# barbararoessle/e2e_multi_view_matching

Measured on AMD Instinct MI355X. Metric: image-pairs/sec @1024 kpts + pose AUC@5/10/20deg vs reference, higher is better.
Workload: dtype f16x2 (fp32 operands carried as 2 fp16 planes hi + 2^-11 lo', 22 significant bits, 3 fp16-MFMA products, fp32 accumulate; same 1e-4 / bit-exact-index parity bar); 1 GPU; configs[1]: tuple_size=2 (1 pair per tuple), 1024 keypoints, 256-dim f32 descriptors, GNN 9x1 = 18 layers, 100 Sinkhorn iters, batch 32 tuples/GPU = 32 pairs/GPU, w8pt pose per pair; pairs_per_gpu=32, global_pairs=32, weights=random init (timed), identity-like for the AUC leg, parallelism=tuple-sharded x1

## Files before the change

### e2e_multi_view_matching_amd/csrc/gemm_p2.hip

```cpp
#include <algorithm>
#include <cstdlib>
#include <type_traits>

#include "gemm_p2_core.h"

namespace e2emv {

template <int OUT, bool HAS_R = false>
__global__ __launch_bounds__(512, 1) void gemm_p2_kernel(GemmP2Params p) {
    extern __shared__ __attribute__((aligned(16))) char smem_p2[];

    const int xcd = blockIdx.x & 7, slot = blockIdx.x >> 3, slots = gridDim.x >> 3;
    const int per_xcd = (p.total + 7) / 8;
    const int t_begin = xcd * per_xcd;
    const int t_end = min(t_begin + per_xcd, p.total);
    int tile = t_begin + slot;
    if (tile >= t_end) return;

    const int tid = threadIdx.x, lane = tid & 63;
    const int wave = __builtin_amdgcn_readfirstlane(tid >> 6);
    const int wr = wave >> 1, wc = wave & 1;
    const int l31 = lane & 31, lh = lane >> 5;
    const int nk = p.K / P2_BK, nk1 = p.K1 / P2_BK;

    const __amdgpu_buffer_rsrc_t rsA = __builtin_amdgcn_make_buffer_rsrc(const_cast<uint16_t*>(p.A), 0, (int)p.a_bytes, 0x00020000);
    const __amdgpu_buffer_rsrc_t rsA2 = __builtin_amdgcn_make_buffer_rsrc(const_cast<uint16_t*>(p.A2), 0, (int)p.a2_bytes, 0x00020000);
    const __amdgpu_buffer_rsrc_t rsW = __builtin_amdgcn_make_buffer_rsrc(const_cast<uint16_t*>(p.W), 0, (int)p.w_bytes, 0x00020000);

    const int ld_r = lane >> 3, ld_p = lane & 7;
    unsigned a_vo[4], a2_vo[4], w_vo[4];
    auto setup = [&](int t) {
        const int tm = t / p.tiles_n, tn = t - tm * p.tiles_n;
#pragma unroll
        for (int i = 0; i < 4; ++i) {
            const int row = 32 * wave + 8 * i + ld_r;
            const unsigned c = (unsigned)(ld_p ^ ((row >> 1) & 7));
            const unsigned gm = (unsigned)min(tm * P2_BM + row, p.M - 1);
            a_vo[i] = gm * p.lda_b + c * 16u;
            a2_vo[i] = gm * p.lda2_b + c * 16u;
            const unsigned gn = (unsigned)min(tn * P2_BN + row, p.N - 1);
            w_vo[i] = gn * p.ldw_b + c * 16u;
        }
    };
    auto issue = [&](int buf, int kt, unsigned dep) {
        char* dst = smem_p2 + buf * P2_BUFB + 32 * wave * P2_ROWB;
        if (kt < nk1) {
            const unsigned so = (unsigned)kt * 128u;
#pragma unroll
            for (int i = 0; i < 4; ++i) p2_glds16(rsA, dst + i * 1024, a_vo[i] + dep, so);
        } else {
            const unsigned so = (unsigned)(kt - nk1) * 128u;
#pragma unroll
            for (int i = 0; i < 4; ++i) p2_glds16(rsA2, dst + i * 1024, a2_vo[i] + dep, so);
        }
        const unsigned sw = (unsigned)kt * 128u;
#pragma unroll
        for (int i = 0; i < 4; ++i) p2_glds16(rsW, dst + P2_TILEB + i * 1024, w_vo[i] + dep, sw);
    };

    const int swz = (l31 >> 1) & 7;
    p2_f32x16 acc[4][2];



    int ld_tile = tile, ld_kt = 0;
    bool ld_valid = true;
    auto advance = [&]() {
        if (ld_kt + 1 < nk) { ++ld_kt; return; }
        if (ld_tile + slots < t_end) {
            ld_tile += slots;
            ld_kt = 0;
            setup(ld_tile);
        } else {
            ld_valid = false;
        }
    };
    setup(tile);
    issue(0, 0, 0u);
    advance();
    const bool issue_first = wave >= 4;
    const bool overlap = nk >= 3;
    const bool has_e = p.EA != nullptr || (HAS_R && p.ER != nullptr);
    int e_run = 0, cur_kt = 0;
    int ev = 0, ev_next = 0;
    auto fetch_e = [&](int t) {
        int v = 0;
        if (has_e) {
            const int tm_ = t / p.tiles_n, tn_ = t - tm_ * p.tiles_n;
            const int erow = tm_ * 4 + wr;
            const int nb1 = nk1 >> 1, nb = (nk + 1) >> 1;
            if (erow * 64 < p.M) {
                if (lane < nb) {
                    if (p.EA) v = lane < nb1 ? p.EA[erow * p.eld_a + lane] : (p.EA2 ? p.EA2[erow * p.eld_a2 + lane - nb1] : 0);
                } else if (HAS_R && p.ER && lane >= 32 && lane < 36) {
                    const int cb = tn_ * 4 + wc * 2 + (lane & 1);
                    if (cb < p.eld_r) {
                        if (lane < 34) v = p.ER[erow * p.eld_r + cb];
                        else if (p.AR) v = __builtin_bit_cast(int, p.AR[erow * p.eld_r + cb]);
                    }
                }
            }
        }
        return v;
    };
    ev = fetch_e(tile);
    int since = 8;
    bool ahead = false;
    int buf = 0;
    auto step = [&](auto FIRST) {
        if (since == 0 && ahead) asm volatile("s_waitcnt vmcnt(40)" ::: "memory");
        else if (since <= 1 && overlap) asm volatile("s_waitcnt vmcnt(32)" ::: "memory");
        else asm volatile("s_waitcnt vmcnt(0)" ::: "memory");
        asm volatile("s_waitcnt lgkmcnt(0)\n\ts_barrier" ::: "memory");
        if (has_e) {
            const int e_step = p.EA ? __builtin_amdgcn_readlane(ev, cur_kt >> 1) : 0;
            if (!decltype(FIRST)::value && e_step != e_run) {
                asm volatile("s_nop 15");
                const int d = e_run - e_step;
                const float f = d < -126 ? 0.f : p2_exp2i(d);
#pragma unroll
                for (int j = 0; j < 4; ++j)
#pragma unroll
                    for (int i = 0; i < 2; ++i)
#pragma unroll
                        for (int r = 0; r < 16; ++r) acc[j][i][r] *= f;
            }
            e_run = e_step;
            if (nk >= 4 && tile + slots < t_end) {
                if (cur_kt == 2) ev_next = fetch_e(tile + slots);
                if (cur_kt == 3) asm volatile("" : "+v"(ev_next));
            }
        }
        ++cur_kt;
        const bool ldv = ld_valid && !(since == 0 && ahead);
        if (issue_first && ldv) issue(buf ^ 1, ld_kt, 0u);
        gp_kstep<decltype(FIRST)::value>(smem_p2, buf, wr, wc, l31, lh, acc);
        if (!issue_first && ldv) {
            unsigned dep = 0;
            asm("" : "+v"(dep) : "v"(acc[3][1]));
            issue(buf ^ 1, ld_kt, dep);
        }
        if (ldv) advance();
        if (since == 0) ahead = false;
        ++since;
        buf ^= 1;
    };
    for (;;) {
        step(std::true_type{});
        for (int kt = 1; kt < nk; ++kt) step(std::false_type{});
        if (overlap && ld_valid) {
            asm volatile("s_waitcnt lgkmcnt(0)\n\ts_barrier" ::: "memory");
            unsigned dep = 0;
            asm("" : "+v"(dep) : "v"(acc[3][1]));
            issue(buf ^ 1, ld_kt, dep);
            advance();
            ahead = true;
        }
        cur_kt = 0;
        if (has_e && nk < 4 && tile + slots < t_end) ev_next = fetch_e(tile + slots);
        gp_acc_fence(acc);
        gp_epilogue<OUT, HAS_R>(p, smem_p2, acc, wave, tile / p.tiles_n, tile % p.tiles_n, e_run, ev);
        ev = ev_next;
        since = overlap ? 0 : 8;
        tile += slots;
        if (tile >= t_end) break;
    }
}

int fill_gemm_p2_params(e2emv_ctx* ctx, const GemmP2Args& a, GemmP2Params& p) {
    if (a.M <= 0 || a.N <= 0 || a.K <= 0) return set_err(ctx, E2EMV_ESHAPE, "gemm_p2: empty problem");
    const int K1 = a.A2 ? a.K1 : a.K;
    if (a.K % 32 || K1 % 32 || K1 <= 0 || K1 > a.K || (K1 < a.K && !a.A2))
        return set_err(ctx, E2EMV_ESHAPE, "gemm_p2: K=%d K1=%d must be multiples of 32", a.K, K1);
    if (!a.A || !a.W || a.lda % 32 || a.lda < K1 || (a.A2 && (a.lda2 % 32 || a.lda2 < a.K - K1)))
        return set_err(ctx, E2EMV_ESHAPE, "gemm_p2: operand planes need whole 32-column blocks (lda=%lld lda2=%lld)", (long long)a.lda, (long long)a.lda2);
    if ((uintptr_t)a.A % 16 || (a.A2 && (uintptr_t)a.A2 % 16) || (uintptr_t)a.W % 16 || (a.bias && (uintptr_t)a.bias % 16) || (a.Rp && (uintptr_t)a.Rp % 16))
        return set_err(ctx, E2EMV_ESHAPE, "gemm_p2: operands must be 16-byte aligned");
    if (a.Rp && (a.ldr % 32 || a.ldr < a.N)) return set_err(ctx, E2EMV_ESHAPE, "gemm_p2: residual planes need ldr %% 32 == 0");
    const int64_t a_bytes = (int64_t)a.M * a.lda * 4, a2_bytes = a.A2 ? (int64_t)a.M * a.lda2 * 4 : 16, w_bytes = (int64_t)a.N * a.K * 4;
    if (a_bytes >= ((int64_t)1 << 31) || a2_bytes >= ((int64_t)1 << 31) || w_bytes >= ((int64_t)1 << 31))
        return set_err(ctx, E2EMV_ESHAPE, "gemm_p2: operand larger than 2 GB (M=%d lda=%lld): 32-bit byte offsets", a.M, (long long)a.lda);
    p = GemmP2Params{};
    p.A = a.A; p.A2 = a.A2 ? a.A2 : a.A; p.W = a.W;
    p.a_bytes = (unsigned)a_bytes; p.a2_bytes = (unsigned)(a.A2 ? a2_bytes : a_bytes); p.w_bytes = (unsigned)w_bytes;
    p.lda_b = (unsigned)(a.lda * 4); p.lda2_b = (unsigned)((a.A2 ? a.lda2 : a.lda) * 4); p.ldw_b = (unsigned)(a.K * 4);
    p.bias = a.bias; p.Rp = a.Rp; p.ldr = a.ldr;
// ... 61 lines not shown
```

### e2e_multi_view_matching_amd/csrc/gemm_p2_core.h

```cpp
#pragma once
#include <type_traits>

#include "p2.h"

namespace e2emv {

typedef __attribute__((ext_vector_type(16))) float p2_f32x16;

constexpr int P2_BM = 256, P2_BN = 256, P2_BK = 32;
constexpr int P2_ROWB = 128;
constexpr int P2_TILEB = P2_BM * P2_ROWB;
constexpr int P2_BUFB = 2 * P2_TILEB;
constexpr int P2_SLABB = 32 * 32 * 4;
constexpr int P2_LDSB = 2 * P2_BUFB + 8 * P2_SLABB;

struct GemmP2Params {
    const uint16_t* A;
    const uint16_t* A2;
    const uint16_t* W;
    unsigned a_bytes, a2_bytes, w_bytes;
    unsigned lda_b, lda2_b, ldw_b;
    const float* bias;
    const uint16_t* Rp;
    float* C32;
    uint16_t* Cp;
    uint16_t* Vt;
    int64_t ldc, ldr;
    int M, N, K, K1;
    int tiles_n, total, relu;
    float out_scale;
    float col_scale[3];
    int n_rows, heads;
    const int* EA;
    const int* EA2;
    const int* ER;
    int* EC;
    int* EVt;
    const float* AR;
    float* AC;
    int eld_a, eld_a2, eld_r, eld_c;
    float bias_amax;
    unsigned* stats;
    char* dummy;
};

__device__ __forceinline__ int gp_lane_now() {
    int l;
    asm volatile("v_mbcnt_lo_u32_b32 %0, -1, 0\n\tv_mbcnt_hi_u32_b32 %0, -1, %0" : "=v"(l));
    return l;
}

int fill_gemm_p2_params(e2emv_ctx* ctx, const GemmP2Args& a, GemmP2Params& p);

__device__ __forceinline__ void gp_mfma(p2_f32x16& c, p2_f16x8 a, p2_f16x8 b) {
    asm volatile("v_mfma_f32_32x32x16_f16 %0, %1, %2, %0" : "+v"(c) : "v"(a), "v"(b));
}
__device__ __forceinline__ void gp_mfma0(p2_f32x16& c, p2_f16x8 a, p2_f16x8 b) {
    asm volatile("v_mfma_f32_32x32x16_f16 %0, %1, %2, 0" : "=&v"(c) : "v"(a), "v"(b));
}
__device__ __forceinline__ unsigned gp_pk_mul(unsigned x, unsigned k) {
    unsigned d;
    asm volatile("v_pk_mul_f16 %0, %1, %2" : "=v"(d) : "v"(x), "v"(k));
    return d;
}

__device__ __forceinline__ float gp_amax3(float a, float x, float y) {
    asm("v_max3_f32 %0, %0, |%1|, |%2|" : "+v"(a) : "v"(x), "v"(y));
    return a;
}
__device__ __forceinline__ void gp_relu2x8(p2_f32x4& v0, p2_f32x4& v1, int on) {
    float a = v0[0], b = v0[1], c = v0[2], d = v0[3], e = v1[0], f = v1[1], g = v1[2], h = v1[3];
    asm("s_cmp_eq_u32 %8, 0\n\t"
        "s_cbranch_scc1 1f\n\t"
        "v_add_f32_e64 %0, %0, |%0|\n\t"
        "v_add_f32_e64 %1, %1, |%1|\n\t"
        "v_add_f32_e64 %2, %2, |%2|\n\t"
        "v_add_f32_e64 %3, %3, |%3|\n\t"
        "v_add_f32_e64 %4, %4, |%4|\n\t"
        "v_add_f32_e64 %5, %5, |%5|\n\t"
        "v_add_f32_e64 %6, %6, |%6|\n\t"
        "v_add_f32_e64 %7, %7, |%7|\n"
        "1:"
        : "+v"(a), "+v"(b), "+v"(c), "+v"(d), "+v"(e), "+v"(f), "+v"(g), "+v"(h) : "s"(on) : "scc");
    v0 = p2_f32x4{a, b, c, d};
    v1 = p2_f32x4{e, f, g, h};
}
__device__ __forceinline__ p2_f32x2 gp_join_scaled(unsigned hi, unsigned lo) {
    float x0, x1;
    asm("v_fma_mix_f32 %0, %2, %4, %3 op_sel_hi:[1,0,1]\n\tv_fma_mix_f32 %1, %2, %4, %3 op_sel:[1,0,1] op_sel_hi:[1,0,1]"
        : "=&v"(x0), "=&v"(x1) : "v"(lo), "v"(hi), "s"(1.f / 2048.f));
    return {x0, x1};
}
template <bool SCALED>
__device__ __forceinline__ void gp_split8(const p2_f32x4& a0, const p2_f32x4& a1, const p2_f32x4& b0, const p2_f32x4& b1, p2_u32x4& hi, p2_u32x4& lo) {
    const p2_f32x2 q0 = {a0[0], a0[1]}, q1 = {a0[2], a0[3]}, q2 = {a1[0], a1[1]}, q3 = {a1[2], a1[3]};
    const unsigned h0 = __builtin_bit_cast(unsigned, __builtin_convertvector(q0, p2_f16x2)), h1 = __builtin_bit_cast(unsigned, __builtin_convertvector(q1, p2_f16x2));
    const unsigned h2 = __builtin_bit_cast(unsigned, __builtin_convertvector(q2, p2_f16x2)), h3 = __builtin_bit_cast(unsigned, __builtin_convertvector(q3, p2_f16x2));
    unsigned l0, l1, l2, l3;
    asm("v_fma_mixlo_f16 %0, %4, %16, %8 op_sel_hi:[1,0,0]\n\t"
        "v_fma_mixlo_f16 %1, %5, %16, %10 op_sel_hi:[1,0,0]\n\t"
        "v_fma_mixlo_f16 %2, %6, %16, %12 op_sel_hi:[1,0,0]\n\t"
        "v_fma_mixlo_f16 %3, %7, %16, %14 op_sel_hi:[1,0,0]\n\t"
        "v_fma_mixhi_f16 %0, %4, %16, %9 op_sel:[1,0,0] op_sel_hi:[1,0,0]\n\t"
        "v_fma_mixhi_f16 %1, %5, %16, %11 op_sel:[1,0,0] op_sel_hi:[1,0,0]\n\t"
        "v_fma_mixhi_f16 %2, %6, %16, %13 op_sel:[1,0,0] op_sel_hi:[1,0,0]\n\t"
        "v_fma_mixhi_f16 %3, %7, %16, %15 op_sel:[1,0,0] op_sel_hi:[1,0,0]\n\t"
        "s_nop 1"
        : "=&v"(l0), "=&v"(l1), "=&v"(l2), "=&v"(l3)
        : "v"(h0), "v"(h1), "v"(h2), "v"(h3), "v"(b0[0]), "v"(b0[1]), "v"(b0[2]), "v"(b0[3]), "v"(b1[0]), "v"(b1[1]), "v"(b1[2]), "v"(b1[3]),
          "s"(SCALED ? -2048.f : -1.f));
    hi = p2_u32x4{h0, h1, h2, h3};
    lo = p2_u32x4{l0, l1, l2, l3};
}

template <bool first_step>
__device__ __forceinline__ void gp_kstep(const char* smem, int buf, int wr, int wc, int l31, int lh, p2_f32x16 (&acc)[4][2]) {
    const int swz = (l31 >> 1) & 7;
    const char* xs = smem + buf * P2_BUFB + (wr * 64 + l31) * P2_ROWB;
    const char* ws = smem + buf * P2_BUFB + P2_TILEB + (wc * 128 + l31) * P2_ROWB;
    auto rd_x = [&](int ks, int t, int pl) { return *reinterpret_cast<const p2_f16x8*>(xs + t * 32 * P2_ROWB + (((4 * pl + 2 * ks + lh) ^ swz) << 4)); };
    auto rd_w = [&](int ks, int j, int pl) { return *reinterpret_cast<const p2_f16x8*>(ws + j * 32 * P2_ROWB + (((4 * pl + 2 * ks + lh) ^ swz) << 4)); };
    p2_f16x8 xb[2][2][2];
    p2_f16x8 wb[2][2];
    unsigned k2048 = 0x10001000u;
    asm volatile("" : "+v"(k2048));
#pragma unroll
    for (int t = 0; t < 2; ++t)
#pragma unroll
        for (int pl = 0; pl < 2; ++pl) xb[0][t][pl] = rd_x(0, t, pl);
    wb[0][1] = rd_w(0, 0, 1);
    wb[0][0] = rd_w(0, 0, 0);
    __builtin_amdgcn_sched_barrier(0);
#pragma unroll
    for (int g = 0; g < 8; ++g) {
        const int ks = g >> 2, j = g & 3, gp = g & 1;
        const p2_u32x4 wh = __builtin_bit_cast(p2_u32x4, wb[gp][0]);
        p2_u32x4 w2u;
        const bool z = first_step && ks == 0;
        if (z) gp_mfma0(acc[j][0], wb[gp][1], xb[ks][0][0]); else gp_mfma(acc[j][0], wb[gp][1], xb[ks][0][0]);
#pragma unroll
        for (int e = 0; e < 4; ++e) w2u[e] = gp_pk_mul(wh[e], k2048);
        __builtin_amdgcn_sched_barrier(0);
        if (z) gp_mfma0(acc[j][1], wb[gp][1], xb[ks][1][0]); else gp_mfma(acc[j][1], wb[gp][1], xb[ks][1][0]);
        if (g < 7) {
            wb[gp ^ 1][1] = rd_w((g + 1) >> 2, (g + 1) & 3, 1);
            wb[gp ^ 1][0] = rd_w((g + 1) >> 2, (g + 1) & 3, 0);
        }
        __builtin_amdgcn_sched_barrier(0);
        const p2_f16x8 w2 = __builtin_bit_cast(p2_f16x8, w2u);
        gp_mfma(acc[j][0], w2, xb[ks][0][1]);
        if (ks == 0 && j == 2) { xb[1][0][0] = rd_x(1, 0, 0); xb[1][1][0] = rd_x(1, 1, 0); }
        __builtin_amdgcn_sched_barrier(0);
        gp_mfma(acc[j][1], w2, xb[ks][1][1]);
        if (ks == 0 && j == 3) { xb[1][0][1] = rd_x(1, 0, 1); xb[1][1][1] = rd_x(1, 1, 1); }
        __builtin_amdgcn_sched_barrier(0);
        gp_mfma(acc[j][0], wb[gp][0], xb[ks][0][0]);
        __builtin_amdgcn_sched_barrier(0);
        gp_mfma(acc[j][1], wb[gp][0], xb[ks][1][0]);
        __builtin_amdgcn_sched_barrier(0);
    }
}

__device__ __forceinline__ void gp_acc_fence(p2_f32x16 (&acc)[4][2]) {
    asm volatile("s_nop 15" : "+v"(acc[0][0]), "+v"(acc[0][1]), "+v"(acc[1][0]), "+v"(acc[1][1]), "+v"(acc[2][0]), "+v"(acc[2][1]), "+v"(acc[3][0]), "+v"(acc[3][1]));
}

template <int OUT, bool HAS_R, bool RLDS = false>
__device__ __forceinline__ void gp_epilogue(const GemmP2Params& p, char* smem, const p2_f32x16 (&acc)[4][2], int wave, int tm, int tn, int e_run, int ev) {
    static_assert(!RLDS || (HAS_R && OUT == P2_OUT_PLANES), "the LDS residual ring belongs to the plane epilogue with a residual");
    const int lane = gp_lane_now();
    const int wr = wave >> 1, wc = wave & 1;
    const int l31 = lane & 31, lh = lane >> 5;
    char* sl = smem + 2 * P2_BUFB + wave * P2_SLABB;
    const int o_r = lane >> 2, o_c = (lane & 3) * 8;
    const int o_z = o_r & 7;
    const float cs = OUT == P2_OUT_QKV ? p.col_scale[min(tn, 2)] : 1.f;
    char* dummy = p.dummy + lane * 64;
    const float os = p.out_scale * p2_exp2i(e_run);
    const int erow = tm * 4 + wr;
    float rsc[2] = {1.f, 1.f};
    float osc[2] = {1.f, 1.f};
    float iosc[2] = {1.f, 1.f};
    float amx[2][2] = {{0.f, 0.f}, {0.f, 0.f}};
    if ((OUT != P2_OUT_F32 && (p.EC || p.EVt)) || (HAS_R && p.ER)) {
#pragma unroll
        for (int ch = 0; ch < 2; ++ch) {
            const int cb = tn * 4 + wc * 2 + ch;
            int er = 0;
            float ar = 0.f;
            if (HAS_R && p.ER) {
                er = __builtin_amdgcn_readlane(ev, 32 + ch);
                ar = p.AR ? __builtin_bit_cast(float, __builtin_amdgcn_readlane(ev, 34 + ch)) : 65536.f * p2_exp2i(er);
            }
            rsc[ch] = p2_exp2i(er);
            int* E = (OUT == P2_OUT_QKV && tn == 2) ? p.EVt : p.EC;
            if (OUT == P2_OUT_F32 || !E) continue;
            float am = 0.f, am1 = 0.f;
#pragma unroll
            for (int i = 0; i < 2; ++i)
#pragma unroll
                for (int jj = 0; jj < 2; ++jj)
#pragma unroll
                    for (int r = 0; r < 16; r += 4) {
                        am = gp_amax3(am, acc[2 * ch + jj][i][r], acc[2 * ch + jj][i][r + 1]);
                        am1 = gp_amax3(am1, acc[2 * ch + jj][i][r + 2], acc[2 * ch + jj][i][r + 3]);
                    }
            am = p2_wave_max(fmaxf(am, am1));
            const float bound = am * os + p.bias_amax + ar;
            const int e = p2_pick_exponent(bound * cs);
            osc[ch] = p2_exp2i(-e);
            iosc[ch] = p2_exp2i(e);
            const int ecb = (OUT == P2_OUT_QKV && tn == 2) ? wc * 2 + ch : cb;
            const int eld = (OUT == P2_OUT_QKV && tn == 2) ? 4 : p.eld_c;
            if (lane == 0 && erow * 64 < p.M && ecb < eld) {
                E[erow * eld + ecb] = e;
                if (e != 0 && p.stats) atomicAdd(p.stats, 1u);
            }
        }
    }
    const unsigned sw0 = (unsigned)(uintptr_t)(__attribute__((address_space(3))) char*)sl + (unsigned)(l31 * 128 + ((lh ^ (l31 & 7)) << 4));
    auto slab_write = [&](int i, int j) {
        unsigned a = sw0;
        asm volatile("" : "+v"(a));
#pragma unroll
        for (int g = 0; g < 4; ++g) {
            p2_f32x4 v;
#pragma unroll
            for (int e = 0; e < 4; ++e) v[e] = acc[j][i][4 * g + e];
            typedef __attribute__((address_space(3))) p2_f32x4* lds_f32x4_t;
            *reinterpret_cast<lds_f32x4_t>((uintptr_t)(a ^ (32u * g))) = v;
        }
    };
    if (OUT == P2_OUT_QKV && tn == 2) {
        const int dl0 = lane >> 2, q = lane & 3;
        const int rb = 16 * (q >> 1) + 4 * (q & 1);
        float vb[4][2];
#pragma unroll
        for (int j = 0; j < 4; ++j)
#pragma unroll
            for (int pass = 0; pass < 2; ++pass) {
                const int n = tn * P2_BN + wc * 128 + j * 32 + dl0 + 16 * pass;
                vb[j][pass] = (p.bias && n < p.N) ? p.bias[n] : 0.f;
            }
        const unsigned vt_rd0 = (unsigned)(uintptr_t)(__attribute__((address_space(3))) char*)sl
                                + (unsigned)(rb * 128 + ((((dl0 >> 2) ^ (rb & 7)) << 4) | ((dl0 & 3) << 2)));
        const int64_t row2 = 2 * (int64_t)p.n_rows;
        uint16_t* const vt_lane = p.Vt + dl0 * row2 + q * 8;
#pragma unroll
        for (int i = 0; i < 2; ++i) {
            const int m0 = tm * P2_BM + wr * 64 + i * 32;
            const int img = m0 / p.n_rows, key0 = m0 - img * p.n_rows;
            const int64_t off_i = (int64_t)img * p.heads * 64 * row2 + (key0 >> 5) * 64;
#pragma unroll
            for (int j = 0; j < 4; ++j) {
                slab_write(i, j);
                const float f = cs * osc[j >> 1], of = os * f;
#pragma unroll
                for (int pass = 0; pass < 2; ++pass) {
                    const int dl = dl0 + 16 * pass;
                    unsigned a0 = vt_rd0 ^ (pass ? 64u : 0u);
                    asm volatile("" : "+v"(a0));
                    float v[8];
#pragma unroll
                    for (int t = 0; t < 4; ++t) {
// ... 41 lines not shown
    }
    auto rl_issue = [&](int bb) {
        if constexpr (RLDS) {
            const int i = bb >> 2, j = bb & 3;
            const unsigned m0 = (unsigned)(tm * P2_BM + wr * 64 + i * 32);
            const unsigned so = m0 * (unsigned)p.ldr * 4u + (unsigned)(tn * 8 + wc * 4 + j) * 128u;
            asm volatile("" ::: "memory");
#pragma unroll
            for (int q = 0; q < 4; ++q) p2_glds16(rsR, rl_base + (bb & 3) * 4096 + q * 1024, rl_vo, so + (unsigned)q * 8u * (unsigned)p.ldr * 4u);
            asm volatile("" ::: "memory");
        }
    };
    if constexpr (RLDS) {
#pragma unroll
        for (int bb = 0; bb < 4; ++bb) rl_issue(bb);
    }
    p2_f32x4 rv[2][2][2];
    p2_u32x4 rr[RREG ? 2 : 1][2][2];
    const int row0 = tm * P2_BM + wr * 64 + o_r, col0 = tn * P2_BN + wc * 128 + o_c;
    const int rows_left = p.M - row0;
    const int64_t rstep = (OUT == P2_OUT_F32 ? 16 : 32) * p.ldc;
    float* const c32_t = OUT == P2_OUT_F32 ? p.C32 + (int64_t)row0 * p.ldc + col0 : nullptr;
    uint16_t* const cp_t = OUT == P2_OUT_F32 ? nullptr : p.Cp + p2_index(row0, col0, p.ldc);
    const bool relu = OUT != P2_OUT_QKV && p.relu;
    const bool fold = relu && OUT == P2_OUT_PLANES && !HAS_R;
    const float unfold = relu && !fold ? 0.5f : 1.f;
    auto stage = [&](auto BB) {
        constexpr int b = decltype(BB)::value;
        constexpr int i = b >> 2, j = b & 3;
        slab_write(i, j);
        if (RREG) load_bias(b & 1, j);
        const uint16_t* rcol = nullptr;
        if constexpr (RREG) {
            const int nc = min(col0 + j * 32, p.N - 8);
            rcol = p.Rp + ((nc >> 5) * 64 + (nc & 31));
        }
#pragma unroll
        for (int pass = 0; pass < 2; ++pass) {
            const int r = o_r + 16 * pass;
            const int c0 = 2 * (lane & 3);
            rv[b & 1][pass][0] = *reinterpret_cast<const p2_f32x4*>(sl + r * 128 + ((c0 ^ o_z) << 4));
            rv[b & 1][pass][1] = *reinterpret_cast<const p2_f32x4*>(sl + r * 128 + (((c0 + 1) ^ o_z) << 4));
            if constexpr (RREG) {
                int m = min(row0 + i * 32 + 16 * pass, p.M - 1);
                const uint16_t* rp = rcol + (int64_t)m * (2 * p.ldr);
                rr[b & 1][pass][0] = *reinterpret_cast<const p2_u32x4*>(rp);
                rr[b & 1][pass][1] = *reinterpret_cast<const p2_u32x4*>(rp + 32);
            }
        }
    };
    auto finish = [&](auto BB) {
        constexpr int b = decltype(BB)::value;
        constexpr int i = b >> 2, j = b & 3;
        const bool col_ok = col0 + j * 32 < p.N;
        const float fa = OUT == P2_OUT_F32 ? 1.f : cs * osc[j >> 1] * (fold ? 0.5f : 1.f);
        float osf = os, rsf = 1.f;
        if constexpr (HAS_R) rsf = rsc[j >> 1];
        p2_u32x4 rq[2][2];
        if constexpr (RLDS) {
            constexpr int CNT[8] = {12, 16, 20, 24, 28, 24, 20, 16};
            asm volatile("s_waitcnt vmcnt(%0)" :: "n"(CNT[b]) : "memory");
            const unsigned sw = (((unsigned)o_r >> 1) & 1u) << 2;
#pragma unroll
            for (int pass = 0; pass < 2; ++pass) {
                const char* rp_ = rl_base + (b & 3) * 4096 + (o_r + 16 * pass) * 128;
                rq[pass][0] = *reinterpret_cast<const p2_u32x4*>(rp_ + ((((unsigned)lane & 3u) ^ sw) << 4));
                rq[pass][1] = *reinterpret_cast<const p2_u32x4*>(rp_ + (((4u + ((unsigned)lane & 3u)) ^ sw) << 4));
// ... 77 lines not shown
```

### e2e_multi_view_matching_amd/csrc/gemm_p2c.hip

```cpp
#include <algorithm>
#include <cstdlib>

#include "gemm_p2_core.h"

namespace e2emv {

constexpr int P2C_MAX_STAGES = 4, P2C_MAX_TILES = 16;
constexpr int P2C_INDEP = P2_CHAIN_INDEP;

struct GemmP2ChainParams {
    GemmP2Params st[P2C_MAX_STAGES];
    int kind[P2C_MAX_STAGES];
    int dep_kt[P2C_MAX_STAGES];
    int first[P2C_MAX_STAGES + 1];
    int n_stages, row_blocks;
    int t_info[P2C_MAX_TILES];
};

__global__ __launch_bounds__(512, 1) void gemm_p2_chain_kernel(GemmP2ChainParams cp_by_value) {
    extern __shared__ __attribute__((aligned(16))) char smem_p2c[];
    (void)cp_by_value;
    const GemmP2ChainParams& cp = *(const GemmP2ChainParams*)(const __attribute__((address_space(4))) GemmP2ChainParams*)__builtin_amdgcn_kernarg_segment_ptr();

    const int wave = __builtin_amdgcn_readfirstlane(threadIdx.x >> 6);
    const int wr = wave >> 1, wc = wave & 1;
    int l31 = 0, lh = 0;
    unsigned rc_t = 0;
    const int nst = cp.n_stages, tpr = cp.first[nst];
    const int n_my = (cp.row_blocks - (int)blockIdx.x + (int)gridDim.x - 1) / (int)gridDim.x;
    const int total = n_my * tpr;
    if (total <= 0) return;
    auto is_hard = [&](int f) { return f > 0 && (cp.t_info[f % tpr] & (1 << 16)) != 0; };

    unsigned a_base = 0, w_base = 0;
    unsigned lda_l = 0, ldw_l = 0;
    __amdgpu_buffer_rsrc_t rsA, rsA2, rsW;
    int nk_l = 0, nk1_l = 0;
    auto setup = [&](int f) {
        const int rbi = f / tpr, r = f - rbi * tpr, ti = cp.t_info[r], s = ti & 255;
        const int tm = (int)blockIdx.x + rbi * (int)gridDim.x, tn = (ti >> 8) & 255;
        const GemmP2Params& q = cp.st[s];
        rsA = __builtin_amdgcn_make_buffer_rsrc(const_cast<uint16_t*>(q.A), 0, (int)q.a_bytes, 0x00020000);
        rsA2 = __builtin_amdgcn_make_buffer_rsrc(const_cast<uint16_t*>(q.A2), 0, (int)q.a2_bytes, 0x00020000);
        rsW = __builtin_amdgcn_make_buffer_rsrc(const_cast<uint16_t*>(q.W), 0, (int)q.w_bytes, 0x00020000);
        nk_l = q.K / P2_BK;
        nk1_l = q.K1 / P2_BK;
        lda_l = q.lda_b;
        ldw_l = q.ldw_b;
        a_base = ((unsigned)tm * P2_BM + 32u * wave) * lda_l;
        w_base = ((unsigned)tn * P2_BN + 32u * wave) * ldw_l;
    };
    auto lane_rc = [&]() {
        const unsigned ln = (unsigned)gp_lane_now(), ld_r = ln >> 3, ld_p = ln & 7;
        return ld_r | ((ld_p ^ (ld_r >> 1)) * 16u) << 8;
    };
    auto issue = [&](int buf, int kt, unsigned rc) {
        char* dst = smem_p2c + buf * P2_BUFB + 32 * wave * P2_ROWB;
        const unsigned ld_r = rc & 255u, c16 = rc >> 8;
        const unsigned a0 = __umul24(ld_r, lda_l) + c16, a1 = a0 ^ 64u, w0 = __umul24(ld_r, ldw_l) + c16, w1 = w0 ^ 64u;
// ... 18 lines not shown
        p2_glds16(rsW, dst + P2_TILEB + 3072, w1, sw + 3 * w_step);
    };

    typedef int p2c_i4 __attribute__((ext_vector_type(4)));
    typedef int p2c_i2 __attribute__((ext_vector_type(2)));
    auto sload4 = [](const int* p) {
        p2c_i4 r;
        asm volatile("s_load_dwordx4 %0, %1, 0x0\n\ts_waitcnt lgkmcnt(0)" : "=&s"(r) : "s"(p) : "memory");
        return r;
    };
    auto sload2 = [](const int* p) {
        p2c_i2 r;
        asm volatile("s_load_dwordx2 %0, %1, 0x0\n\ts_waitcnt lgkmcnt(0)" : "=&s"(r) : "s"(p) : "memory");
        return r;
    };
    auto pack4 = [](p2c_i4 v) { return (unsigned)((v[0] & 255) | (v[1] & 255) << 8 | (v[2] & 255) << 16 | (v[3] & 255) << 24); };
    auto fetch_ew = [&](int f, bool low, bool high, unsigned long long old) {
        const int rbi = f / tpr, r = f - rbi * tpr, ti = cp.t_info[r], s = ti & 255;
        const int erow = ((int)blockIdx.x + rbi * (int)gridDim.x) * 4 + wr;
        const GemmP2Params& q = cp.st[s];
        if (!q.EA) return 0ull;
        const int nb1 = (q.K1 / P2_BK) >> 1, nb = (q.K / P2_BK + 1) >> 1;
        unsigned lo = (unsigned)old, hi = (unsigned)(old >> 32);
        if (low) lo = pack4(sload4(q.EA + erow * q.eld_a));
        if (high) {
            hi = 0;
            if (nb1 == 8) hi = pack4(sload4(q.EA + erow * q.eld_a + 4));
            else if (nb > nb1 && q.EA2) hi = pack4(sload4(q.EA2 + erow * q.eld_a2));
        }
        return (unsigned long long)hi << 32 | lo;
    };
    auto e_of = [](unsigned long long ew, int kb) { return (int)(signed char)(ew >> (8 * kb)); };

    p2_f32x16 acc[4][2];
    int lf = 0, lkt = 0;
    bool ld_valid = true, ld_blocked = false;
    auto advance = [&]() {
        if (__builtin_expect(lkt + 1 < nk_l, 1)) { ++lkt; return; }
        if (lf + 1 >= total) { ld_valid = false; return; }
        if (is_hard(lf + 1)) { ld_blocked = true; return; }
        ++lf;
        lkt = 0;
        setup(lf);
    };
    setup(0);
    issue(0, 0, lane_rc());
    advance();
    unsigned long long ew = fetch_ew(0, true, true, 0), ew_next = 0;
    int er_c[2] = {0, 0}, ar_c[2] = {0, 0};
    const bool issue_first = wave >= 4;
    int e_run = 0, cur_kt = 0;
    int since = 8;
    bool ahead = false;
    int buf = 0;
    bool has_e = false, soft = false, prefetch_next = false;
    int f = 0;
    auto step = [&](auto FIRST) {
        if (since == 0 && ahead) asm volatile("s_waitcnt vmcnt(40)" ::: "memory");
        else if (since <= 1) asm volatile("s_waitcnt vmcnt(32)" ::: "memory");
        else asm volatile("s_waitcnt vmcnt(0)" ::: "memory");
        asm volatile("s_waitcnt lgkmcnt(0)\n\ts_barrier" ::: "memory");
        if (has_e && (cur_kt & 1) == 0) {
            if (__builtin_expect(soft && cur_kt == 4, 0)) {
                asm volatile("s_dcache_inv\n\tbuffer_inv sc0\n\ts_waitcnt lgkmcnt(0)" ::: "memory");
                ew = fetch_ew(f, false, true, ew);
            }
            const int e_step = e_of(ew, cur_kt >> 1);
            if (!decltype(FIRST)::value && __builtin_expect(e_step != e_run, 0)) {
                asm volatile("s_nop 15");
                const int d = e_run - e_step;
                const float fs = d < -126 ? 0.f : p2_exp2i(d);
#pragma unroll
                for (int j = 0; j < 4; ++j)
#pragma unroll
                    for (int i = 0; i < 2; ++i)
#pragma unroll
                        for (int r = 0; r < 16; ++r) acc[j][i][r] *= fs;
            }
            e_run = e_step;
            if (__builtin_expect(cur_kt == 2, 0)) {
                if (prefetch_next) ew_next = fetch_ew(f + 1, true, true, 0);
                const int rr_ = f % tpr, ti_ = cp.t_info[rr_], s_ = ti_ & 255;
                const GemmP2Params& q_ = cp.st[s_];
                if ((cp.kind[s_] & 4) && q_.ER) {
                    const int erow = ((int)blockIdx.x + (f / tpr) * (int)gridDim.x) * 4 + wr;
                    const int cb = ((ti_ >> 8) & 255) * 4 + wc * 2;
                    const p2c_i2 e2 = sload2(q_.ER + erow * q_.eld_r + cb);
                    er_c[0] = e2[0]; er_c[1] = e2[1];
                    if (q_.AR) {
                        const p2c_i2 a2 = sload2(reinterpret_cast<const int*>(q_.AR) + erow * q_.eld_r + cb);
                        ar_c[0] = a2[0]; ar_c[1] = a2[1];
                    }
                }
            }
        }
        ++cur_kt;
        const bool ldv = ld_valid && !ld_blocked && !(since == 0 && ahead);
        if (issue_first && ldv) issue(buf ^ 1, lkt, rc_t);
        gp_kstep<decltype(FIRST)::value>(smem_p2c, buf, wr, wc, l31, lh, acc);
        if (!issue_first && ldv) {
            unsigned rc = rc_t;
            asm("" : "+v"(rc) : "v"(acc[3][1]));
            issue(buf ^ 1, lkt, rc);
        }
        if (ldv) advance();
        if (since == 0) ahead = false;
        ++since;
        buf ^= 1;
    };
    for (f = 0; f < total; ++f) {
        const int rbi = f / tpr, r = f - rbi * tpr, ti = cp.t_info[r], s = ti & 255;
        const int tm = (int)blockIdx.x + rbi * (int)gridDim.x, tn = (ti >> 8) & 255;
        const GemmP2Params& q = cp.st[s];
        const int nk = q.K / P2_BK;
        {
            const int ln = gp_lane_now();
            l31 = ln & 31;
            lh = ln >> 5;
            rc_t = lane_rc();
        }
        has_e = q.EA != nullptr || ((cp.kind[s] & 4) && q.ER != nullptr);
        soft = f > 0 && (ti & (1 << 17)) != 0;
        prefetch_next = f + 1 < total && !is_hard(f + 1);
        step(std::true_type{});
        for (int kt = 1; kt < nk; ++kt) step(std::false_type{});
        if (ld_valid && !ld_blocked) {
            asm volatile("s_waitcnt lgkmcnt(0)\n\ts_barrier" ::: "memory");
            unsigned rc = lane_rc();
            asm("" : "+v"(rc) : "v"(acc[3][1]));
            issue(buf ^ 1, lkt, rc);
            advance();
            ahead = true;
        }
        cur_kt = 0;
        gp_acc_fence(acc);
        int ev = 0;
        if ((cp.kind[s] & 4) && q.ER) {
            asm("v_writelane_b32 %0, %1, 32\n\tv_writelane_b32 %0, %2, 33\n\tv_writelane_b32 %0, %3, 34\n\tv_writelane_b32 %0, %4, 35"
                : "+v"(ev) : "s"(er_c[0]), "s"(er_c[1]), "s"(ar_c[0]), "s"(ar_c[1]));
        }
        switch (cp.kind[s]) {
            case P2_OUT_PLANES: gp_epilogue<P2_OUT_PLANES, false>(q, smem_p2c, acc, wave, tm, tn, e_run, ev); break;
            case P2_OUT_PLANES | 4:
                if (ld_blocked) {
                    asm volatile("s_waitcnt lgkmcnt(0)\n\ts_barrier" ::: "memory");
                    gp_epilogue<P2_OUT_PLANES, true, true>(q, smem_p2c, acc, wave, tm, tn, e_run, ev);
                } else {
                    gp_epilogue<P2_OUT_PLANES, true>(q, smem_p2c, acc, wave, tm, tn, e_run, ev);
                }
                break;
            case P2_OUT_QKV: gp_epilogue<P2_OUT_QKV, false>(q, smem_p2c, acc, wave, tm, tn, e_run, ev); break;
            default: gp_epilogue<P2_OUT_F32, false>(q, smem_p2c, acc, wave, tm, tn, e_run, ev); break;
        }
        ew = ew_next;
        since = 0;
        if (ld_blocked) {
            asm volatile("s_waitcnt vmcnt(0) lgkmcnt(0)\n\ts_barrier\n\tbuffer_inv sc0" ::: "memory");
            ld_blocked = false;
            ++lf;
            lkt = 0;
            setup(lf);
            asm volatile("s_dcache_inv\n\ts_waitcnt lgkmcnt(0)" ::: "memory");
// ... 53 lines not shown
```

Measured before the change: 3321 pairs/s.

## Switch P2 GEMM core from 32x32x16 to 16x16x32 MFMA tiles

Replaces the 32x32x16 f16 MFMA with 16x16x32, changing the accumulator layout to an 8x4 array of f32x4 fragments. The k-step LDS read pattern, swizzle and scheduling are rewritten to match, and the epilogue amax and slab writes are adapted to the new fragment layout. The aim is better MFMA throughput and latency hiding by covering the full 32-deep K slice in one instruction per fragment, at the cost of more MFMA issues, more LDS fragment reads and a different register allocation. It also adds a readfirstlane on the picked exponent and a profiling script that reports effective clock per kernel.

```diff
diff --git a/e2e_multi_view_matching_amd/csrc/gemm_p2.hip b/e2e_multi_view_matching_amd/csrc/gemm_p2.hip
--- a/e2e_multi_view_matching_amd/csrc/gemm_p2.hip
+++ b/e2e_multi_view_matching_amd/csrc/gemm_p2.hip
@@ -20,7 +20,6 @@
     const int tid = threadIdx.x, lane = tid & 63;
     const int wave = __builtin_amdgcn_readfirstlane(tid >> 6);
     const int wr = wave >> 1, wc = wave & 1;
-    const int l31 = lane & 31, lh = lane >> 5;
     const int nk = p.K / P2_BK, nk1 = p.K1 / P2_BK;
 
     const __amdgpu_buffer_rsrc_t rsA = __builtin_amdgcn_make_buffer_rsrc(const_cast<uint16_t*>(p.A), 0, (int)p.a_bytes, 0x00020000);
@@ -58,8 +57,7 @@
         for (int i = 0; i < 4; ++i) p2_glds16(rsW, dst + P2_TILEB + i * 1024, w_vo[i] + dep, sw);
     };
 
-    const int swz = (l31 >> 1) & 7;
-    p2_f32x16 acc[4][2];
+    p2_acc_t acc;
 
 
 
@@ -119,11 +117,11 @@
                 const int d = e_run - e_step;
                 const float f = d < -126 ? 0.f : p2_exp2i(d);
 #pragma unroll
-                for (int j = 0; j < 4; ++j)
-#pragma unroll
-                    for (int i = 0; i < 2; ++i)
-#pragma unroll
-                        for (int r = 0; r < 16; ++r) acc[j][i][r] *= f;
+                for (int j = 0; j < P2_ACC_J; ++j)
+#pragma unroll
+                    for (int i = 0; i < P2_ACC_I; ++i)
+#pragma unroll
+                        for (int r = 0; r < 4; ++r) acc[j][i][r] *= f;
             }
             e_run = e_step;
             if (nk >= 4 && tile + slots < t_end) {
@@ -134,10 +132,10 @@
         ++cur_kt;
         const bool ldv = ld_valid && !(since == 0 && ahead);
         if (issue_first && ldv) issue(buf ^ 1, ld_kt, 0u);
-        gp_kstep<decltype(FIRST)::value>(smem_p2, buf, wr, wc, l31, lh, acc);
+        gp_kstep<decltype(FIRST)::value>(smem_p2, buf, wr, wc, lane, acc);
         if (!issue_first && ldv) {
             unsigned dep = 0;
-            asm("" : "+v"(dep) : "v"(acc[3][1]));
+            asm("" : "+v"(dep) : "v"(acc[P2_ACC_J - 1][P2_ACC_I - 1]));
             issue(buf ^ 1, ld_kt, dep);
         }
         if (ldv) advance();
@@ -151,7 +149,7 @@
         if (overlap && ld_valid) {
             asm volatile("s_waitcnt lgkmcnt(0)\n\ts_barrier" ::: "memory");
             unsigned dep = 0;
-            asm("" : "+v"(dep) : "v"(acc[3][1]));
+            asm("" : "+v"(dep) : "v"(acc[P2_ACC_J - 1][P2_ACC_I - 1]));
             issue(buf ^ 1, ld_kt, dep);
             advance();
             ahead = true;
diff --git a/e2e_multi_view_matching_amd/csrc/gemm_p2_core.h b/e2e_multi_view_matching_amd/csrc/gemm_p2_core.h
--- a/e2e_multi_view_matching_amd/csrc/gemm_p2_core.h
+++ b/e2e_multi_view_matching_amd/csrc/gemm_p2_core.h
@@ -5,7 +5,8 @@
 
 namespace e2emv {
 
-typedef __attribute__((ext_vector_type(16))) float p2_f32x16;
+constexpr int P2_ACC_J = 8, P2_ACC_I = 4;
+typedef p2_f32x4 p2_acc_t[P2_ACC_J][P2_ACC_I];
 
 constexpr int P2_BM = 256, P2_BN = 256, P2_BK = 32;
 constexpr int P2_ROWB = 128;
@@ -52,11 +53,11 @@
 
 int fill_gemm_p2_params(e2emv_ctx* ctx, const GemmP2Args& a, GemmP2Params& p);
 
-__device__ __forceinline__ void gp_mfma(p2_f32x16& c, p2_f16x8 a, p2_f16x8 b) {
-    asm volatile("v_mfma_f32_32x32x16_f16 %0, %1, %2, %0" : "+v"(c) : "v"(a), "v"(b));
-}
-__device__ __forceinline__ void gp_mfma0(p2_f32x16& c, p2_f16x8 a, p2_f16x8 b) {
-    asm volatile("v_mfma_f32_32x32x16_f16 %0, %1, %2, 0" : "=&v"(c) : "v"(a), "v"(b));
+__device__ __forceinline__ void gp_mfma(p2_f32x4& c, p2_f16x8 a, p2_f16x8 b) {
+    asm volatile("v_mfma_f32_16x16x32_f16 %0, %1, %2, %0" : "+v"(c) : "v"(a), "v"(b));
+}
+__device__ __forceinline__ void gp_mfma0(p2_f32x4& c, p2_f16x8 a, p2_f16x8 b) {
+    asm volatile("v_mfma_f32_16x16x32_f16 %0, %1, %2, 0" : "=&v"(c) : "v"(a), "v"(b));
 }
 __device__ __forceinline__ unsigned gp_pk_mul(unsigned x, unsigned k) {
     unsigned d;
@@ -114,63 +115,71 @@
 }
 
 template <bool first_step>
-__device__ __forceinline__ void gp_kstep(const char* smem, int buf, int wr, int wc, int l31, int lh, p2_f32x16 (&acc)[4][2]) {
-    const int swz = (l31 >> 1) & 7;
-    const char* xs = smem + buf * P2_BUFB + (wr * 64 + l31) * P2_ROWB;
-    const char* ws = smem + buf * P2_BUFB + P2_TILEB + (wc * 128 + l31) * P2_ROWB;
-    auto rd_x = [&](int ks, int t, int pl) { return *reinterpret_cast<const p2_f16x8*>(xs + t * 32 * P2_ROWB + (((4 * pl + 2 * ks + lh) ^ swz) << 4)); };
-    auto rd_w = [&](int ks, int j, int pl) { return *reinterpret_cast<const p2_f16x8*>(ws + j * 32 * P2_ROWB + (((4 * pl + 2 * ks + lh) ^ swz) << 4)); };
-    p2_f16x8 xb[2][2][2];
+__device__ __forceinline__ void gp_kstep(const char* smem, int buf, int wr, int wc, int lane, p2_acc_t& acc) {
+    const int l15 = lane & 15, lq = lane >> 4;
+    const int swz = l15 >> 1;
+    const char* xs = smem + buf * P2_BUFB + (wr * 64 + l15) * P2_ROWB;
+    const char* ws = smem + buf * P2_BUFB + P2_TILEB + (wc * 128 + l15) * P2_ROWB;
+    auto rd_x = [&](int t, int pl) { return *reinterpret_cast<const p2_f16x8*>(xs + t * 16 * P2_ROWB + (((4 * pl + lq) ^ swz) << 4)); };
+    auto rd_w = [&](int j, int pl) { return *reinterpret_cast<const p2_f16x8*>(ws + j * 16 * P2_ROWB + (((4 * pl + lq) ^ swz) << 4)); };
+    p2_f16x8 xb[4][2];
     p2_f16x8 wb[2][2];
     unsigned k2048 = 0x10001000u;
     asm volatile("" : "+v"(k2048));
-#pragma unroll
-    for (int t = 0; t < 2; ++t)
-#pragma unroll
-        for (int pl = 0; pl < 2; ++pl) xb[0][t][pl] = rd_x(0, t, pl);
-    wb[0][1] = rd_w(0, 0, 1);
-    wb[0][0] = rd_w(0, 0, 0);
+    xb[0][0] = rd_x(0, 0);
+    wb[0][1] = rd_w(0, 1);
+    xb[1][0] = rd_x(1, 0);
+    wb[0][0] = rd_w(0, 0);
+    xb[2][0] = rd_x(2, 0);
+    xb[3][0] = rd_x(3, 0);
     __builtin_amdgcn_sched_barrier(0);
 #pragma unroll
     for (int g = 0; g < 8; ++g) {
-        const int ks = g >> 2, j = g & 3, gp = g & 1;
+        const int gp = g & 1;
         const p2_u32x4 wh = __builtin_bit_cast(p2_u32x4, wb[gp][0]);
         p2_u32x4 w2u;
-        const bool z = first_step && ks == 0;
-        if (z) gp_mfma0(acc[j][0], wb[gp][1], xb[ks][0][0]); else gp_mfma(acc[j][0], wb[gp][1], xb[ks][0][0]);
+        if (first_step) gp_mfma0(acc[g][0], wb[gp][1], xb[0][0]); else gp_mfma(acc[g][0], wb[gp][1], xb[0][0]);
 #pragma unroll
         for (int e = 0; e < 4; ++e) w2u[e] = gp_pk_mul(wh[e], k2048);
+        if (g == 0) { xb[0][1] = rd_x(0, 1); xb[1][1] = rd_x(1, 1); }
         __builtin_amdgcn_sched_barrier(0);
-        if (z) gp_mfma0(acc[j][1], wb[gp][1], xb[ks][1][0]); else gp_mfma(acc[j][1], wb[gp][1], xb[ks][1][0]);
+        if (first_step) gp_mfma0(acc[g][1], wb[gp][1], xb[1][0]); else gp_mfma(acc[g][1], wb[gp][1], xb[1][0]);
         if (g < 7) {
-            wb[gp ^ 1][1] = rd_w((g + 1) >> 2, (g + 1) & 3, 1);
-            wb[gp ^ 1][0] = rd_w((g + 1) >> 2, (g + 1) & 3, 0);
-        }
+            wb[gp ^ 1][1] = rd_w(g + 1, 1);
+            wb[gp ^ 1][0] = rd_w(g + 1, 0);
+        }
+        __builtin_amdgcn_sched_barrier(0);
+        if (first_step) gp_mfma0(acc[g][2], wb[gp][1], xb[2][0]); else gp_mfma(acc[g][2], wb[gp][1], xb[2][0]);
+        if (g == 0) { xb[2][1] = rd_x(2, 1); xb[3][1] = rd_x(3, 1); }
+        __builtin_amdgcn_sched_barrier(0);
+        if (first_step) gp_mfma0(acc[g][3], wb[gp][1], xb[3][0]); else gp_mfma(acc[g][3], wb[gp][1], xb[3][0]);
         __builtin_amdgcn_sched_barrier(0);
         const p2_f16x8 w2 = __builtin_bit_cast(p2_f16x8, w2u);
-        gp_mfma(acc[j][0], w2, xb[ks][0][1]);
-        if (ks == 0 && j == 2) { xb[1][0][0] = rd_x(1, 0, 0); xb[1][1][0] = rd_x(1, 1, 0); }
-        __builtin_amdgcn_sched_barrier(0);
-        gp_mfma(acc[j][1], w2, xb[ks][1][1]);
-        if (ks == 0 && j == 3) { xb[1][0][1] = rd_x(1, 0, 1); xb[1][1][1] = rd_x(1, 1, 1); }
-        __builtin_amdgcn_sched_barrier(0);
-        gp_mfma(acc[j][0], wb[gp][0], xb[ks][0][0]);
-        __builtin_amdgcn_sched_barrier(0);
-        gp_mfma(acc[j][1], wb[gp][0], xb[ks][1][0]);
-        __builtin_amdgcn_sched_barrier(0);
-    }
-}
-
-__device__ __forceinline__ void gp_acc_fence(p2_f32x16 (&acc)[4][2]) {
-    asm volatile("s_nop 15" : "+v"(acc[0][0]), "+v"(acc[0][1]), "+v"(acc[1][0]), "+v"(acc[1][1]), "+v"(acc[2][0]), "+v"(acc[2][1]), "+v"(acc[3][0]), "+v"(acc[3][1]));
+#pragma unroll
+        for (int i = 0; i < 4; ++i) {
+            gp_mfma(acc[g][i], w2, xb[i][1]);
+            __builtin_amdgcn_sched_barrier(0);
+        }
+#pragma unroll
+        for (int i = 0; i < 4; ++i) {
+            gp_mfma(acc[g][i], wb[gp][0], xb[i][0]);
+            __builtin_amdgcn_sched_barrier(0);
+        }
+    }
+}
+
+__device__ __forceinline__ void gp_acc_fence(p2_acc_t& acc) {
+    asm volatile("s_nop 15" : "+v"(acc[0][0]), "+v"(acc[0][1]), "+v"(acc[0][2]), "+v"(acc[0][3]), "+v"(acc[1][0]), "+v"(acc[1][1]), "+v"(acc[1][2]), "+v"(acc[1][3]),
+                              "+v"(acc[2][0]), "+v"(acc[2][1]), "+v"(acc[2][2]), "+v"(acc[2][3]), "+v"(acc[3][0]), "+v"(acc[3][1]), "+v"(acc[3][2]), "+v"(acc[3][3]));
+    asm volatile("s_nop 15" : "+v"(acc[4][0]), "+v"(acc[4][1]), "+v"(acc[4][2]), "+v"(acc[4][3]), "+v"(acc[5][0]), "+v"(acc[5][1]), "+v"(acc[5][2]), "+v"(acc[5][3]),
+                              "+v"(acc[6][0]), "+v"(acc[6][1]), "+v"(acc[6][2]), "+v"(acc[6][3]), "+v"(acc[7][0]), "+v"(acc[7][1]), "+v"(acc[7][2]), "+v"(acc[7][3]));
 }
 
 template <int OUT, bool HAS_R, bool RLDS = false>
-__device__ __forceinline__ void gp_epilogue(const GemmP2Params& p, char* smem, const p2_f32x16 (&acc)[4][2], int wave, int tm, int tn, int e_run, int ev) {
+__device__ __forceinline__ void gp_epilogue(const GemmP2Params& p, char* smem, const p2_acc_t& acc, int wave, int tm, int tn, int e_run, int ev) {
     static_assert(!RLDS || (HAS_R && OUT == P2_OUT_PLANES), "the LDS residual ring belongs to the plane epilogue with a residual");
     const int lane = gp_lane_now();
     const int wr = wave >> 1, wc = wave & 1;
-    const int l31 = lane & 31, lh = lane >> 5;
     char* sl = smem + 2 * P2_BUFB + wave * P2_SLABB;
     const int o_r = lane >> 2, o_c = (lane & 3) * 8;
     const int o_z = o_r & 7;
@@ -197,17 +206,15 @@
             if (OUT == P2_OUT_F32 || !E) continue;
             float am = 0.f, am1 = 0.f;
 #pragma unroll
-            for (int i = 0; i < 2; ++i)
-#pragma unroll
-                for (int jj = 0; jj < 2; ++jj)
-#pragma unroll
-                    for (int r = 0; r < 16; r += 4) {
-                        am = gp_amax3(am, acc[2 * ch + jj][i][r], acc[2 * ch + jj][i][r + 1]);
-                        am1 = gp_amax3(am1, acc[2 * ch + jj][i][r + 2], acc[2 * ch + jj][i][r + 3]);
-                    }
+            for (int i = 0; i < P2_ACC_I; ++i)
+#pragma unroll
+                for (int jj = 0; jj < 4; ++jj) {
+                    am = gp_amax3(am, acc[4 * ch + jj][i][0], acc[4 * ch + jj][i][1]);
+                    am1 = gp_amax3(am1, acc[4 * ch + jj][i][2], acc[4 * ch + jj][i][3]);
+                }
             am = p2_wave_max(fmaxf(am, am1));
             const float bound = am * os + p.bias_amax + ar;
-            const int e = p2_pick_exponent(bound * cs);
+            const int e = __builtin_amdgcn_readfirstlane(p2_pick_exponent(bound * cs));
             osc[ch] = p2_exp2i(-e);
             iosc[ch] = p2_exp2i(e);
             const int ecb = (OUT == P2_OUT_QKV && tn == 2) ? wc * 2 + ch : cb;
@@ -218,18 +225,17 @@
             }
         }
     }
-    const unsigned sw0 = (unsigned)(uintptr_t)(__attribute__((address_space(3))) char*)sl + (unsigned)(l31 * 128 + ((lh ^ (l31 & 7)) << 4));
+    const unsigned sw0 = (unsigned)(uintptr_t)(__attribute__((address_space(3))) char*)sl + (unsigned)((lane & 15) * 128 + (((lane >> 4) ^ (lane & 7)) << 4));
     auto slab_write = [&](int i, int j) {
         unsigned a = sw0;
         asm volatile("" : "+v"(a));
 #pragma unroll
-        for (int g = 0; g < 4; ++g) {
-            p2_f32x4 v;
-#pragma unroll
-            for (int e = 0; e < 4; ++e) v[e] = acc[j][i][4 * g + e];
-            typedef __attribute__((address_space(3))) p2_f32x4* lds_f32x4_t;
-            *reinterpret_cast<lds_f32x4_t>((uintptr_t)(a ^ (32u * g))) = v;
-        }
+        for (int ra = 0; ra < 2; ++ra)
+#pragma unroll
+            for (int cb = 0; cb < 2; ++cb) {
+                typedef __attribute__((address_space(3))) p2_f32x4* lds_f32x4_t;
+                *reinterpret_cast<lds_f32x4_t>((uintptr_t)((a ^ (64u * cb)) + 2048u * ra)) = acc[2 * j + cb][2 * i + ra];
+            }
     };
     if (OUT == P2_OUT_QKV && tn == 2) {
         const int dl0 = lane >> 2, q = lane & 3;
@@ -337,7 +343,8 @@
         if (RREG) load_bias(b & 1, j);
         const uint16_t* rcol = nullptr;
         if constexpr (RREG) {
-            const int nc = min(col0 + j * 32, p.N - 8);
+            int nc = min(col0 + j * 32, p.N - 8);
+            asm volatile("" : "+v"(nc));
             rcol = p.Rp + ((nc >> 5) * 64 + (nc & 31));
         }
 #pragma unroll
diff --git a/e2e_multi_view_matching_amd/csrc/gemm_p2c.hip b/e2e_multi_view_matching_amd/csrc/gemm_p2c.hip
--- a/e2e_multi_view_matching_amd/csrc/gemm_p2c.hip
+++ b/e2e_multi_view_matching_amd/csrc/gemm_p2c.hip
@@ -24,7 +24,7 @@
 
     const int wave = __builtin_amdgcn_readfirstlane(threadIdx.x >> 6);
     const int wr = wave >> 1, wc = wave & 1;
-    int l31 = 0, lh = 0;
+    int lane_t = 0;
     unsigned rc_t = 0;
     const int nst = cp.n_stages, tpr = cp.first[nst];
     const int n_my = (cp.row_blocks - (int)blockIdx.x + (int)gridDim.x - 1) / (int)gridDim.x;
@@ -109,7 +109,7 @@
     };
     auto e_of = [](unsigned long long ew, int kb) { return (int)(signed char)(ew >> (8 * kb)); };
 
-    p2_f32x16 acc[4][2];
+    p2_acc_t acc;
     int lf = 0, lkt = 0;
     bool ld_valid = true, ld_blocked = false;
     auto advance = [&]() {
@@ -148,11 +148,11 @@
                 const int d = e_run - e_step;
                 const float fs = d < -126 ? 0.f : p2_exp2i(d);
 #pragma unroll
-                for (int j = 0; j < 4; ++j)
+                for (int j = 0; j < P2_ACC_J; ++j)
 #pragma unroll
-                    for (int i = 0; i < 2; ++i)
+                    for (int i = 0; i < P2_ACC_I; ++i)
 #pragma unroll
-                        for (int r = 0; r < 16; ++r) acc[j][i][r] *= fs;
+                        for (int r = 0; r < 4; ++r) acc[j][i][r] *= fs;
             }
             e_run = e_step;
             if (__builtin_expect(cur_kt == 2, 0)) {
@@ -174,10 +174,10 @@
         ++cur_kt;
         const bool ldv = ld_valid && !ld_blocked && !(since == 0 && ahead);
         if (issue_first && ldv) issue(buf ^ 1, lkt, rc_t);
-        gp_kstep<decltype(FIRST)::value>(smem_p2c, buf, wr, wc, l31, lh, acc);
+        gp_kstep<decltype(FIRST)::value>(smem_p2c, buf, wr, wc, lane_t, acc);
         if (!issue_first && ldv) {
             unsigned rc = rc_t;
-            asm("" : "+v"(rc) : "v"(acc[3][1]));
+            asm("" : "+v"(rc) : "v"(acc[P2_ACC_J - 1][P2_ACC_I - 1]));
             issue(buf ^ 1, lkt, rc);
         }
         if (ldv) advance();
@@ -191,9 +191,7 @@
         const GemmP2Params& q = cp.st[s];
         const int nk = q.K / P2_BK;
         {
-            const int ln = gp_lane_now();
-            l31 = ln & 31;
-            lh = ln >> 5;
+            lane_t = gp_lane_now();
             rc_t = lane_rc();
         }
         has_e = q.EA != nullptr || ((cp.kind[s] & 4) && q.ER != nullptr);
@@ -204,7 +202,7 @@
         if (ld_valid && !ld_blocked) {
             asm volatile("s_waitcnt lgkmcnt(0)\n\ts_barrier" ::: "memory");
             unsigned rc = lane_rc();
-            asm("" : "+v"(rc) : "v"(acc[3][1]));
+            asm("" : "+v"(rc) : "v"(acc[P2_ACC_J - 1][P2_ACC_I - 1]));
             issue(buf ^ 1, lkt, rc);
             advance();
             ahead = true;
diff --git a/profiles/pmc_clock.py b/profiles/pmc_clock.py
--- /dev/null
+++ b/profiles/pmc_clock.py
@@ -0,0 +1,25 @@
+import collections
+import csv
+import glob
+import sys
+
+
+def main():
+    d, subs = sys.argv[1], sys.argv[2:]
+    rows = collections.defaultdict(list)
+    for f in glob.glob(d + "/**/*counter_collection*.csv", recursive=True):
+        with open(f) as fh:
+            for r in csv.DictReader(fh):
+                name = r.get("Kernel_Name", "?")
+                if r.get("Counter_Name") != "GRBM_GUI_ACTIVE" or (subs and not any(s in name for s in subs)):
+                    continue
+                rows[name].append((float(r["Counter_Value"]), float(r["End_Timestamp"]) - float(r["Start_Timestamp"])))
+    for name, v in rows.items():
+        v = [x for x in v if x[1] > 3e5] or v
+        ghz = sorted(c / 8 / w for c, w in v)
+        print("%-90s n=%3d wall %8.1f us  clock GHz min %.3f med %.3f max %.3f"
+              % (name[:90], len(v), sum(w for _, w in v) / len(v) / 1e3, ghz[0], ghz[len(ghz) // 2], ghz[-1]))
+
+
+if __name__ == "__main__":
+    main()
```

Measured after the change: 3362 pairs/s, median of 6. 1.01x the previous value.
